# arnauqb/GradABM-JUNE

Hardware: AMD Instinct MI355X
Metric: simulation steps/sec (higher is better)
Workload: dtype f32

## Files before the change

### gradabm-june_amd/csrc/gj_tiled.h

```cpp
#pragma once
#include <hip/hip_runtime.h>
#include <stdint.h>

#include <type_traits>

#include "../../include/gradjune_hip.h"
#include "gj_device.h"

namespace gj {

constexpr int kTileThreads = 1024;
constexpr int kTileWaves = kTileThreads / kWave;
constexpr int kMaxSliceAgents = 19840;
constexpr int kUnroll = 8;
#ifndef GJ_UNROLL_NARROW
#define GJ_UNROLL_NARROW 16
#endif
constexpr int kUnrollNarrow = GJ_UNROLL_NARROW;
#ifndef GJ_VENUE_UNROLL
#define GJ_VENUE_UNROLL 2
#endif
constexpr int kVenueUnroll = GJ_VENUE_UNROLL;
#ifndef GJ_VENUE_UNROLL_C
#define GJ_VENUE_UNROLL_C GJ_VENUE_UNROLL
// ... 389 lines not shown
  for (int pass = 0; pass < 2; ++pass) {
    if (pass == 1 && !two_sources) break;
    bool any = false;
    for (int t = 0; t < A.n_sets; ++t)
      if (A.sets[t].active && !A.sets[t].presum && (!two_sources || A.sets[t].raw == pass)) any = true;
    if (!any) continue;
    if (pass == 1) __syncthreads();
    load_slice(lds_x, pass == 0 ? A.qtrans : A.trans, base, n_local, tid);
    __syncthreads();
    for (int t = 0; t < A.n_sets; ++t) {
      const TSetA& T = A.sets[t];
      if (!T.active || T.presum || (two_sources && T.raw != pass)) continue;
      if (T.wide == 2) {
        scatter_explicit<kUnroll>(T, lds_x, s, wave, lane);
      } else if (T.wide) {
        scatter_set<true>(T, lds_x, s, wave, lane);
      } else {
        scatter_set<false>(T, lds_x, s, wave, lane);
      }
    }
  }
}

struct TSetB {
  const int32_t* blk_v0;
  const int32_t* blk_e0;
  const uint16_t* e_lv;
  const uint8_t* e_cls;
  float* val;
  const float* v_pc;
  float* cum;
  int32_t stride;
  int32_t nk;
  float beta[GJ_MAX_NETS_PER_SET];
  int32_t table[GJ_MAX_NETS_PER_SET];
  int32_t age75[GJ_MAX_NETS_PER_SET];
  int32_t leisure;
  int32_t direct;
  uint32_t term_limit;
  int32_t _pad_b;
  const uint16_t* pv_blk;
  const int32_t* blk_r0;
  const float* x;
  int64_t n_x;
};

struct TileBArgs {
  TSetB sets[GJ_MAX_SETS];
  const int32_t* work;
  const float* tables;
  int32_t day_type;
  int32_t mode;
  int32_t transpose;
  int32_t _pad;
};

struct ClassWeights {
  float l, lw;
};
__device__ __forceinline__ ClassWeights class_weights(const float* tables, int table, int age75, int day_type, int c) {
  const float l = tables[(int64_t)table * GJ_TABLE_SIZE + day_type * 200 + c];
  return {l, age75 ? l * (((c % 100) > 75) ? 1.0f : 0.0f) : l};
}
template <bool TRANSMITTING, bool RECEIVING, typename TSet>
__device__ __forceinline__ void fill_class_weights(float* transmitting, float* receiving, const TSet& T, const float* tables,
                                                   int day_type, int transpose, int tid) {
  for (int i = tid; i < T.nk * 200; i += kTileThreads) {
    const int k = i / 200, c = i % 200;
    const ClassWeights w = class_weights(tables, T.table[k], T.age75[k], day_type, c);
    if (TRANSMITTING) transmitting[i] = transpose ? w.lw : w.l;
    if (RECEIVING) receiving[i] = transpose ? w.l : w.lw;
  }
}

__device__ __noinline__ void venue_group_slow(fx_t* sums, uint32_t* vflags, int words, uint32_t limit, int base_k, int l0,
                                              int l1, int l2, int l3, int l4, int l5, int l6, int l7, float x0, float x1,
                                              float x2, float x3, float x4, float x5, float x6, float x7) {
  const int lv[8] = {l0, l1, l2, l3, l4, l5, l6, l7};
  const float x[8] = {x0, x1, x2, x3, x4, x5, x6, x7};
#pragma unroll
  for (int q = 0; q < 8; ++q) {
    if (lv[q] == 0xFFFF) continue;
    if (abs_bits(x[q]) <= limit) {
      atomicAdd(&sums[base_k + lv[q]], to_fx<kFxVenue>(x[q]));
    } else {
      fx_flag(vflags, words, base_k + lv[q], x[q]);
    }
  }
}

__device__ __forceinline__ int class_byte(uint32_t four, int j) { return (four >> (8 * j)) & 0xFF; }

struct Group8 {
  uint32_t w[4], c[2];
  float v[8];
  __device__ __forceinline__ Group8(uint4 raw, uint2 craw, float4 xa = make_float4(0.0f, 0.0f, 0.0f, 0.0f),
                                    float4 xb = make_float4(0.0f, 0.0f, 0.0f, 0.0f))
      : w{raw.x, raw.y, raw.z, raw.w}, c{craw.x, craw.y}, v{xa.x, xa.y, xa.z, xa.w, xb.x, xb.y, xb.z, xb.w} {}
  __device__ __forceinline__ int lv(int q) const { return (w[q >> 1] >> ((q & 1) * 16)) & 0xFFFF; }
  __device__ __forceinline__ float x(int q) const { return v[q]; }
  __device__ __forceinline__ int cls(int q) const { return class_byte(c[q >> 2], q & 3); }
  __device__ __forceinline__ void drop(int q) { w[q >> 1] |= 0xFFFFu << ((q & 1) * 16); }
  __device__ __forceinline__ bool one_venue() const {
    return (w[0] == w[1]) && (w[1] == w[2]) && (w[2] == w[3]) && ((w[0] >> 16) == (w[0] & 0xFFFFu)) && (lv(0) != 0xFFFF);
  }
  __device__ __forceinline__ Group8 weighted(const float* tk) const {
    Group8 g = *this;
#pragma unroll
    for (int q = 0; q < 8; ++q) g.v[q] = tk[cls(q)] * v[q];
    return g;
  }
};

#ifdef GJ_DIAG_STAMPS
constexpr int kDiagVenueSlots = 8192;
__device__ unsigned long long gj_diag_venue[3 * kDiagVenueSlots];
struct VenueStamp {
  unsigned long long t0;
  __device__ VenueStamp() : t0(__builtin_amdgcn_s_memrealtime()) {}
  __device__ ~VenueStamp() {
    if (threadIdx.x == 0 && blockIdx.x < kDiagVenueSlots) {
      gj_diag_venue[3 * blockIdx.x] = t0;
      gj_diag_venue[3 * blockIdx.x + 1] = __builtin_amdgcn_s_memrealtime();
      gj_diag_venue[3 * blockIdx.x + 2] = __builtin_amdgcn_s_getreg((31 << 11) | 20) & 0xF;
    }
  }
};
#else
struct VenueStamp {};
#endif

struct VenueItem {
  const TSetB& T;
  int tid, nk;
  int v0, nv;
  int g0, g1;
  fx_t* sums;
  float* cumf;
  float* tabs;
  uint32_t* vflags;
  int vwords;
  int dummy;
  __device__ __forceinline__ VenueItem(const TSetB& T_, int j, float* lds, int tid_)
      : T(T_), tid(tid_), nk(T_.nk), v0(T_.blk_v0[j]), nv(T_.blk_v0[j + 1] - v0), g0(T_.blk_e0[j] >> 3),
        g1(T_.blk_e0[j + 1] >> 3), sums(reinterpret_cast<fx_t*>(lds)), cumf(lds), tabs(lds + 2 * ((size_t)nk * nv + 64)),
        vflags(reinterpret_cast<uint32_t*>(tabs + (T_.leisure ? 2 * nk * 200 : 0))), vwords((nk * nv + 64 + 31) / 32),
        dummy(nk * nv + (tid_ & 63)) {}
  __device__ __forceinline__ const uint4* lv8() const { return reinterpret_cast<const uint4*>(T.e_lv); }
  __device__ __forceinline__ const uint2* cls8() const { return reinterpret_cast<const uint2*>(T.e_cls); }
  __device__ __forceinline__ float4* val4() const { return reinterpret_cast<float4*>(T.val); }
};

__device__ __forceinline__ void run_sums(const VenueItem& W, const Group8& G, int base_k, fx_t* sums, uint32_t* vflags) {
  const uint32_t kLimit = W.T.term_limit;
  static_assert(kFxVenue == 36, "term_limit is derived from 2^(50 - kFxVenue) (fill_set_b)");
  if (__builtin_expect(max_abs_bits(G.v) > kLimit, 0)) {
    venue_group_slow(sums, vflags, W.vwords, kLimit, base_k, G.lv(0), G.lv(1), G.lv(2), G.lv(3), G.lv(4), G.lv(5),
                     G.lv(6), G.lv(7), G.x(0), G.x(1), G.x(2), G.x(3), G.x(4), G.x(5), G.x(6), G.x(7));
    return;
  }
  fx_t s8 = 0;
#pragma unroll
  for (int q = 0; q < 8; ++q) {
    const fx_t f = to_fx<kFxVenue>(G.x(q));
    const bool first = (q == 0) || (G.lv(q) != G.lv(q - (q > 0)));
    s8 = first ? f : s8 + f;
    const bool last = (q == 7) || (G.lv(q + (q < 7)) != G.lv(q));
    const bool take = last && G.lv(q) != 0xFFFF;
    atomicAdd(&sums[take ? base_k + G.lv(q) : W.dummy], s8);
  }
}
__device__ __forceinline__ bool one_venue_sum(const VenueItem& W, const Group8& G, int target, fx_t* sums) {
  if (__builtin_amdgcn_ballot_w64(max_abs_bits(G.v) > W.T.term_limit) != 0ull) return false;
  fx_t s = 0;
#pragma unroll
  for (int q = 0; q < 8; ++q) s += to_fx<kFxVenue>(G.x(q));
  s = wave_sum<fx_t>(s);
  if ((W.tid & (kWave - 1)) == 0) atomicAdd(&sums[target], s);
  return true;
}

__device__ __forceinline__ void venue_zero(const VenueItem& W, fx_t* sums, uint32_t* vflags) {
  for (int i = W.tid; i < W.nk * W.nv + 64; i += kTileThreads) sums[i] = 0;
  for (int i = W.tid; i < 2 * W.vwords; i += kTileThreads) vflags[i] = 0u;
}

__device__ __forceinline__ void venue_sums_tiled(const VenueItem& W, const float* weights, fx_t* sums, uint32_t* vflags) {
  const TSetB& T = W.T;
  auto add_group = [&](const Group8& G) {
    const bool mine = G.one_venue() && (G.lv(0) == __builtin_amdgcn_readfirstlane(G.lv(0)));
    const bool one_venue = __builtin_amdgcn_ballot_w64(mine) == ~0ull;
    if (!T.leisure) {
      if (!(one_venue && one_venue_sum(W, G, G.lv(0), sums))) run_sums(W, G, 0, sums, vflags);
    } else {
      for (int k = 0; k < W.nk; ++k) {
        const Group8 Gk = G.weighted(weights + k * 200);
        if (!(one_venue && one_venue_sum(W, Gk, k * W.nv + G.lv(0), sums))) run_sums(W, Gk, k * W.nv, sums, vflags);
      }
    }
  };
  for (int g = W.g0 + W.tid; g < W.g1; g += kVenueUnroll * kTileThreads) {
    uint4 raw[kVenueUnroll];
    float4 xa[kVenueUnroll], xb[kVenueUnroll];
    uint2 craw[kVenueUnroll];
#pragma unroll
    for (int u = 0; u < kVenueUnroll; ++u) {
      const int gu = min(g + u * kTileThreads, W.g1 - 1);
      raw[u] = W.lv8()[gu];
      xa[u] = load_nt(W.val4() + 2 * gu);
      xb[u] = load_nt(W.val4() + 2 * gu + 1);
      craw[u] = T.leisure ? W.cls8()[gu] : make_uint2(0u, 0u);
    }
#pragma unroll
    for (int u = 0; u < kVenueUnroll; ++u)
      if (g + u * kTileThreads < W.g1) add_group(Group8(raw[u], craw[u], xa[u], xb[u]));
  }
}

__device__ __forceinline__ void venue_sums_runs(const VenueItem& W, int j, fx_t* sums, uint32_t* vflags) {
  const TSetB& T = W.T;
  const int r0 = T.blk_r0[j], r1 = T.blk_r0[j + 1];
  const uint4* pv8 = reinterpret_cast<const uint4*>(T.pv_blk);
  const float4* x4 = reinterpret_cast<const float4*>(T.x);
  const int ga = r0 >> 3, gb = (r1 + 7) >> 3;
  const int g_in = (int)(T.n_x >> 3);
  for (int g = ga + W.tid; g < gb; g += kVenueUnroll * kTileThreads) {
    uint4 raw[kVenueUnroll];
    float4 xa[kVenueUnroll], xb[kVenueUnroll];
#pragma unroll
    for (int u = 0; u < kVenueUnroll; ++u) {
      const int gu = min(g + u * kTileThreads, gb - 1);
      raw[u] = pv8[gu];
      if (gu < g_in) {
        xa[u] = x4[2 * gu];
        xb[u] = x4[2 * gu + 1];
      } else {
        float t[8];
#pragma unroll
        for (int q = 0; q < 8; ++q) t[q] = ((int64_t)gu * 8 + q < T.n_x) ? T.x[(int64_t)gu * 8 + q] : 0.0f;
        xa[u] = make_float4(t[0], t[1], t[2], t[3]);
        xb[u] = make_float4(t[4], t[5], t[6], t[7]);
      }
    }
#pragma unroll
    for (int u = 0; u < kVenueUnroll; ++u) {
      const int gu = g + u * kTileThreads;
      if (gu >= gb) continue;
      Group8 G(raw[u], make_uint2(0u, 0u), xa[u], xb[u]);
#pragma unroll
      for (int q = 0; q < 8; ++q) {
        const int a = gu * 8 + q;
        if (!(a >= r0 && a < r1)) G.drop(q);
      }
      run_sums(W, G, 0, sums, vflags);
    }
  }
}

__device__ __forceinline__ void venue_cum_write(const VenueItem& W, const fx_t* sums, const uint32_t* vflags, float* cumf) {
  const TSetB& T = W.T;
  for (int l0 = W.tid; l0 < W.nv; l0 += kCumBatch * kTileThreads) {
    float pc[kCumBatch];
#pragma unroll
    for (int u = 0; u < kCumBatch; ++u) pc[u] = T.v_pc[W.v0 + min(l0 + u * kTileThreads, W.nv - 1)];
    for (int k = 0; k < W.nk; ++k) {
      const float beta = T.beta[k];
#pragma unroll
      for (int u = 0; u < kCumBatch; ++u) {
        const int lv = l0 + u * kTileThreads;
        if (lv < W.nv) {
          const float c = (beta * pc[u]) * fx_read<kFxVenue>(sums, vflags, W.vwords, k * W.nv + lv);
          T.cum[(int64_t)(W.v0 + lv) * T.stride + k] = c;
          cumf[2 * (k * W.nv + lv)] = c;
        }
      }
    }
  }
}
__device__ __forceinline__ void venue_cum_read(const VenueItem& W, float* cumf) {
  const TSetB& T = W.T;
  for (int k = 0; k < W.nk; ++k) {
    for (int l0 = W.tid; l0 < W.nv; l0 += kCumBatch * kTileThreads) {
      float c[kCumBatch];
#pragma unroll
      for (int u = 0; u < kCumBatch; ++u)
        c[u] = T.cum[(int64_t)(W.v0 + min(l0 + u * kTileThreads, W.nv - 1)) * T.stride + k];
#pragma unroll
      for (int u = 0; u < kCumBatch; ++u) {
        const int lv = l0 + u * kTileThreads;
        if (lv < W.nv) cumf[2 * (k * W.nv + lv)] = c[u];
      }
    }
  }
}

__device__ __forceinline__ void venue_gather(const VenueItem& W, const float* weights, const float* cumf) {
  const TSetB& T = W.T;
  const int nk = W.nk, nv = W.nv;
  for (int g = W.g0 + W.tid; g < W.g1; g += kVenueUnrollC * kTileThreads) {
    uint4 raw[kVenueUnrollC];
    uint2 craw[kVenueUnrollC];
#pragma unroll
    for (int u = 0; u < kVenueUnrollC; ++u) {
      const int gu = min(g + u * kTileThreads, W.g1 - 1);
      raw[u] = W.lv8()[gu];
      craw[u] = T.leisure ? W.cls8()[gu] : make_uint2(0u, 0u);
    }
#pragma unroll
    for (int u = 0; u < kVenueUnrollC; ++u) {
      const int gu = g + u * kTileThreads;
      if (gu >= W.g1) continue;
      const Group8 G(raw[u], craw[u]);
      float r[8];
      if (!T.leisure) {
#pragma unroll
        for (int q = 0; q < 8; ++q) {
          const int lv = G.lv(q);
          const float c = cumf[2 * (lv != 0xFFFF ? lv : 0)];
          r[q] = (lv != 0xFFFF) ? c : 0.0f;
        }
      } else {
#pragma unroll
        for (int q = 0; q < 8; ++q) {
          const int lv = G.lv(q);
          const int c = G.cls(q);
          const int li = lv != 0xFFFF ? lv : 0;
          float a = 0.0f;
          for (int k = 0; k < nk; ++k) a += weights[k * 200 + c] * cumf[2 * (k * nv + li)];
          r[q] = (lv != 0xFFFF) ? a : 0.0f;
        }
      }
      store_nt(W.val4() + 2 * gu, make_float4(r[0], r[1], r[2], r[3]));
      store_nt(W.val4() + 2 * gu + 1, make_float4(r[4], r[5], r[6], r[7]));
    }
  }
}

#ifndef GJ_VENUE_WAVES_PER_SIMD
#define GJ_VENUE_WAVES_PER_SIMD 4
#endif
__global__ __launch_bounds__(kTileThreads, GJ_VENUE_WAVES_PER_SIMD) void k_tile_venues(const TileBArgs B) {
  extern __shared__ __align__(16) float lds_s[];
  [[maybe_unused]] const VenueStamp gj_stamp;
  const int set = B.work[2 * blockIdx.x], j = B.work[2 * blockIdx.x + 1];
  const TSetB& T = B.sets[set];
  if (T.nk == 0) return;
  const VenueItem W(T, j, lds_s, threadIdx.x);
  if (T.leisure) fill_class_weights<true, true>(W.tabs, W.tabs + W.nk * 200, T, B.tables, B.day_type, B.transpose, W.tid);
  if (B.mode != 2) {
    venue_zero(W, W.sums, W.vflags);
    __syncthreads();
    venue_sums_tiled(W, W.tabs, W.sums, W.vflags);
    if (T.pv_blk) venue_sums_runs(W, j, W.sums, W.vflags);
    __syncthreads();
    venue_cum_write(W, W.sums, W.vflags, W.cumf);
    if (B.mode == 1 || T.direct) return;
  } else {
    if (T.direct) return;
    venue_cum_read(W, W.cumf);
  }
  __syncthreads();
  venue_gather(W, W.tabs + W.nk * 200, W.cumf);
}

constexpr int GJ_MAX_PRESUM = 6;
constexpr int64_t kPresumBad = (int64_t)0x8000000000000000ll;
struct TPSet {
  const uint16_t* ell;
  int64_t plane_stride;
  fx_t* partial;
  int32_t planes, V, stride, nk;
  int32_t group_venues;
  int32_t raw, leisure, _pad;
  int32_t table[GJ_MAX_NETS_PER_SET];
  int32_t age75[GJ_MAX_NETS_PER_SET];
};
struct TilePArgs {
  TPSet sets[GJ_MAX_PRESUM];
  int32_t n_sets;
  int32_t agents_per_wg;
  int64_t n_agents;
  const float* trans;
  const float* qtrans;
  const uint8_t* cls;
  const float* tables;
  int32_t day_type, transpose;
};

constexpr int kPresumQuads = 3;
__device__ __forceinline__ void fx_add_or_poison(fx_t* sums, uint32_t* flags, int i, float x) {
  const bool ok = fabsf(x) <= fx_max<kFxVenue>();
  atomicAdd(&sums[i], to_fx<kFxVenue>(ok ? x : 0.0f));
  if (__builtin_expect(!ok, 0)) atomicOr(&flags[i >> 5], 1u << (i & 31));
}

__global__ __launch_bounds__(kTileThreads) void k_tile_presum(const TilePArgs P) {
  extern __shared__ __align__(16) fx_t lds_p[];
  const int tid = threadIdx.x;
  const int64_t a_begin = (int64_t)blockIdx.x * P.agents_per_wg;
  const int64_t a_end = min(P.n_agents, a_begin + P.agents_per_wg);
  const int n_quads = (int)((max(a_end - a_begin, (int64_t)0) + 3) >> 2);
  for (int t = 0; t < P.n_sets; ++t) {
    const TPSet& T = P.sets[t];
    const int nk = T.nk;
    const float* x = T.raw ? P.trans : P.qtrans;
    for (int v0 = 0; v0 < T.V; v0 += T.group_venues) {
      const int nv = min(T.group_venues, T.V - v0);
      const int n_sums = nv * nk;
      const int dummy = n_sums + (tid & 63);
      float* wtab = reinterpret_cast<float*>(lds_p + n_sums + 64);
      uint32_t* flags = reinterpret_cast<uint32_t*>(wtab + (T.leisure ? nk * 200 : 0));
      __syncthreads();
      for (int i = tid; i < n_sums + 64; i += kTileThreads) lds_p[i] = 0;
      for (int i = tid; i < (n_sums + 64 + 31) / 32; i += kTileThreads) flags[i] = 0u;
      if (T.leisure) fill_class_weights<true, false>(wtab, nullptr, T, P.tables, P.day_type, P.transpose, tid);
// ... 663 lines not shown
```

### gradabm-june_amd/csrc/gradjune_hip.hip

```cpp
#include <hip/hip_runtime.h>
#include <math.h>
#include <stdint.h>
#include <string.h>

#include "../../include/gradjune_hip.h"
#include "gj_device.h"
#include "gj_tiled.h"
#include "gj_agent.h"

namespace gj {

struct SetP1 {
  const int32_t* v_rowptr;
  const int32_t* v_agent;
  const float* v_pc;
  float* cum;
  int32_t stride;
  int32_t nk;
  float beta[GJ_MAX_NETS_PER_SET];
  int32_t table[GJ_MAX_NETS_PER_SET];
  int32_t raw;
  int32_t leisure;
};

struct P1Args {
  SetP1 sets[GJ_MAX_SETS];
  const gj_block* blocks;
  const float* trans;
  const float* qtrans;
  const uint8_t* cls;
  const float* tables;
  float* partial;
  int32_t day_type;
};

struct SetP2 {
  const int32_t* a_rowptr;
  const int32_t* a_venue;
  const float* cum;
  int32_t stride;
  int32_t nk;
  int32_t mask[GJ_MAX_NETS_PER_SET];
  int32_t table[GJ_MAX_NETS_PER_SET];
};

struct P2Args {
  SetP2 groups[GJ_MAX_SETS];
  int32_t n_groups;
  int32_t any_leisure;
  int64_t n_agents;
  const uint8_t* cls;
  const float* tables;
  const float* stage;
  float* susceptibility;
  float* is_infected;
  float* infection_time;
// ... 773 lines not shown
  for (int g = 0; g < G.n; ++g) {
    const int s = G.set[g];
    if (!uses_presum(plan, s)) continue;
    if (R.n_sets == GJ_MAX_PRESUM) return GJ_E_PLAN;
    PReduceSet& X = R.sets[R.n_sets++];
    const gj_edge_set& E = plan->sets[s];
    X.partial = reinterpret_cast<const fx_t*>(T->sets[s].presum);
    X.v_pc = E.v_pcontact;
    X.cum = E.cum;
    X.V = (int32_t)E.n_venues;
    X.stride = E.cum_stride;
    X.nk = G.nk[g];
    X.first = (int32_t)total;
    const NetGroup C = classify_group(p, G, g);
    memcpy(X.beta, C.beta, sizeof(X.beta));
    total += (int64_t)X.V * X.nk;
  }
  if (R.n_sets == 0 || total == 0) return GJ_OK;
  if (total > INT32_MAX) return GJ_E_RANGE;
  R.total = (int32_t)total;
  return launch(k_presum_reduce, grid_for(total, 0, kWave), kThreads, 0, stream, R);
}

static int tiled_scatter(const gj_plan* plan, const gj_agent_state* st, const gj_step_params* p, const Groups& G,
                         hipStream_t stream) {
  const gj_tiled* T = plan->tiled;
  if (plan->n_ext_agents == 0 || G.n == 0) return GJ_OK;
  TileAArgs A;
  fill_set_a(plan, p, G, A.sets);
  A.n_sets = plan->n_sets;
  A.slice_agents = T->slice_agents;
  A.n_agents = plan->n_ext_agents;
  A.trans = st->transmission;
  A.qtrans = p->has_quarantine ? st->q_transmission : st->transmission;
  const size_t lds = slice_lds(T, sizeof(float));
  int rc = allow_lds(k_tile_scatter, lds);
  if (rc) return rc;
  rc = launch(k_tile_scatter, T->n_slices, kTileThreads, lds, stream, A);
  if (rc) return rc;
  return tiled_presum(plan, st, p, G, stream);
}

static uint32_t venue_term_limit(int32_t max_venue_edges) {
  int e = 14;
  int64_t p2 = 4096;
  while (p2 < (int64_t)max_venue_edges && e > -20) {
    p2 <<= 1;
    --e;
  }
  const float lim = ldexpf(1.0f, e);
  uint32_t bits;
  memcpy(&bits, &lim, sizeof(bits));
  return bits;
}

static int tiled_venues(const gj_plan* plan, const gj_agent_state* st, const gj_step_params* p, const Groups& G, int mode,
                        hipStream_t stream) {
  const gj_tiled* T = plan->tiled;
  if (G.n == 0) return GJ_OK;
  if (T->n_work == 0) return mode == 2 ? GJ_OK : tiled_presum_reduce(plan, p, G, stream);
  TileBArgs B;
  for (int s = 0; s < GJ_MAX_SETS; ++s) B.sets[s] = TSetB{};
  size_t lds = 16;
  for (int g = 0; g < G.n; ++g) {
    const int s = G.set[g];
    const gj_tiled_set& S = T->sets[s];
    const gj_edge_set& E = plan->sets[s];
    TSetB& X = B.sets[s];
    X.blk_v0 = S.blk_v0;
    X.blk_e0 = S.blk_e0;
    X.e_lv = S.e_lv;
    X.e_cls = S.e_cls;
    X.val = S.val;
    X.v_pc = E.v_pcontact;
    X.cum = E.cum;
    X.stride = E.cum_stride;
    X.nk = S.n_blocks > 0 ? G.nk[g] : 0;
    if (uses_presum(plan, s)) X.nk = 0;
    X.direct = S.ell_k != 0;
    const NetGroup C = classify_group(p, G, g);
    X.leisure = C.leisure;
    memcpy(X.beta, C.beta, sizeof(X.beta));
    memcpy(X.table, C.table, sizeof(X.table));
    memcpy(X.age75, C.age75, sizeof(X.age75));
    if (C.leisure && !S.e_cls && E.n_edges > 0) return GJ_E_PLAN;
    if (const int rc = check_group(C)) return rc;
    X.pv_blk = nullptr;
    X.blk_r0 = nullptr;
    X.x = nullptr;
    X.n_x = 0;
    if (S.run_pv_blk && mode != 2) {
      if (X.leisure) return GJ_E_PLAN;
      X.x = (p->has_quarantine && !C.raw) ? st->q_transmission : st->transmission;
      if (!X.x) return GJ_E_NULL;
      if (!aligned16(X.x, S.run_pv_blk)) return GJ_E_PLAN;
      X.pv_blk = S.run_pv_blk;
      X.blk_r0 = S.run_blk_r0;
      X.n_x = plan->n_ext_agents;
    }
    const size_t n_sums = (size_t)X.nk * S.max_block_venues + 64;
    const size_t need = n_sums * sizeof(fx_t) + (X.leisure ? 2 * 200 * (size_t)X.nk : 0) * sizeof(float) +
                        2 * ((n_sums + 31) / 32 * 4);
    X.term_limit = venue_term_limit(S.max_venue_edges);
    if (X.nk && need > lds) lds = need;
  }
  B.work = T->work;
  B.tables = plan->tables;
  B.day_type = p->day_type;
  B.mode = mode;
  B.transpose = p->transpose;
  int rc = allow_lds(k_tile_venues, lds);
  if (rc) return rc;
  rc = launch(k_tile_venues, T->n_work, kTileThreads, lds, stream, B);
  if (rc || mode == 2) return rc;
  return tiled_presum_reduce(plan, p, G, stream);
}

static int tiled_agents(const gj_plan* plan, const gj_agent_state* st, const gj_step_params* p, const Groups& G,
                        const gj_step_io* io, int sample, hipStream_t stream) {
  const gj_tiled* T = plan->tiled;
  if (plan->n_agents == 0) return GJ_OK;
  TileDArgs D;
  fill_set_a(plan, p, G, D.sets);
  D.n_sets = plan->n_sets;
  D.slice_agents = T->slice_agents;
  D.n_agents = plan->n_agents;
  D.stage = st->current_stage;
  D.susceptibility = st->susceptibility;
  D.is_infected = st->is_infected;
  D.infection_time = st->infection_time;
  D.not_infected_probs = io ? io->not_infected_probs : nullptr;
  D.new_infected = io ? io->new_infected : nullptr;
  D.trans_susc = io ? io->trans_susc : nullptr;
  D.agent_sums = io ? io->agent_sums : nullptr;
  D.exp_noise = io ? io->exp_noise : nullptr;
  D.now = p->now;
  D.dt = p->delta_time;
  D.q_thr = p->q_threshold;
  D.has_q = p->has_quarantine;
  D.sample = sample;
  D.seed = p->seed;
  D.step = p->step;
  D.agent_offset = p->agent_offset;
  D.clock = p->clock;
  D.acc_scratch = T->agent_scratch;
  size_t lds = agents_lds(T);
  D.n_direct = 0;
  D.day_type = p->day_type;
  D.transpose = p->transpose;
  D.cls = plan->agent_class;
  D.tables = plan->tables;
  const int64_t owned_slices = (plan->n_agents + T->slice_agents - 1) / T->slice_agents;
  for (int g = 0; g < G.n; ++g) {
    const int s = G.set[g];
    const gj_tiled_set& S = T->sets[s];
    const gj_edge_set& E = plan->sets[s];
    const bool run = S.run_pv_win != nullptr;
    if ((!S.ell_k && !run) || S.n_blocks == 0 || E.n_edges == 0) continue;
    if (D.n_direct == GJ_MAX_DIRECT) return GJ_E_PLAN;
    TDirect& X = D.direct[D.n_direct++];
    X.ell = run ? S.run_pv_win : S.ell;
    X.cum = E.cum;
    X.planes = run ? 1 : S.ell_k / 2;
    X.plane_stride = owned_slices * (int64_t)T->slice_agents * 2;
    X.V = run ? S.run_max_window : (int32_t)E.n_venues;
    X.win_lo = run ? S.run_win_lo : nullptr;
// ... 38 lines not shown
    const size_t direct_lds = 4 * ((size_t)2 * kClassWeightFloats + (size_t)cap0 + kWave + (size_t)cap1 + kWave);
    if (direct_lds > lds) lds = direct_lds;
  }
  D.io_vec4 = aligned16(D.susceptibility, D.not_infected_probs, D.new_infected, D.trans_susc, D.acc_scratch, D.agent_sums);
  int rc = allow_lds(k_tile_agents, lds);
  if (rc) return rc;
  rc = launch(k_tile_agents, owned_slices, kTileThreads, lds, stream, D);
  if (rc || !D.acc_scratch) return rc;
  return launch(k_tile_epilogue, grid_for(plan->n_agents), kThreads, 0, stream, D);
}

static int check_symptoms(const uint8_t* agent_class, const float* new_infected, const float* current_stage,
                          const float* next_stage, const float* time_to_next_stage, const gj_symptoms_params* params,
                          const float* progresses, const float* dwell) {
  if (!agent_class || !new_infected || !current_stage || !next_stage || !time_to_next_stage || !params)
    return GJ_E_NULL;
  if (params->n_stages < 3 || params->n_stages > GJ_MAX_STAGES) return GJ_E_RANGE;
  if ((progresses == nullptr) != (dwell == nullptr)) return GJ_E_NULL;
  if (!progresses && !params->progress) return GJ_E_NULL;
  return GJ_OK;
}

static StatsArgs stats_args(int64_t n, const uint8_t* agent_class, const float* is_infected, const float* current_stage,
                            int32_t n_bins, const int32_t* bin_edges, int32_t dead_stage, double* out, bool vec4) {
  StatsArgs S;
  S.n = n;
  S.cls = agent_class;
  S.inf = is_infected;
  S.stage = current_stage;
  S.n_bins = n_bins;
  for (int b = 0; b <= GJ_MAX_AGE_BINS; ++b) S.edges[b] = (b <= n_bins) ? bin_edges[b] : 0;
  S.dead = dead_stage;
  S.vec4 = (vec4 && (uintptr_t)agent_class % 4 == 0) ? 1 : 0;
  S.out = out;
  return S;
}
static inline int64_t vec4_lanes(int64_t n, int vec4) { return vec4 ? (n >> 2) + 3 : n; }

static int check_profile_adjoint(const gj_agent_state* st, const float* trans_bar, const float* grad_inf_out,
                                 const float* grad_time_inout) {
  if (!st || !trans_bar || !grad_inf_out || !grad_time_inout) return GJ_E_NULL;
  if (!st->max_infectiousness || !st->shape || !st->rate || !st->shift || !st->infection_time || !st->is_infected)
    return GJ_E_NULL;
  return GJ_OK;
}

}


extern "C" {

#ifdef GJ_DIAG_STAMPS
int gj_diag_venue_stamps(unsigned long long* host_out) {
  return (int)hipMemcpyFromSymbol(host_out, HIP_SYMBOL(gj::gj_diag_venue), sizeof(unsigned long long) * 3 * gj::kDiagVenueSlots);
}
#endif

int gj_version(void) { return GJ_ABI_VERSION; }

const char* gj_error_string(int code) {
  switch (code) {
    case GJ_OK: return "ok";
    case GJ_E_NULL: return "required pointer is NULL";
    case GJ_E_RANGE: return "count or index out of range";
    case GJ_E_PLAN: return "inconsistent plan or network list";
    case GJ_E_NODEVICE: return "no HIP device, or not a gfx950 (MI355X) device";
    default: break;
  }
  if (code > 0) return hipGetErrorString((hipError_t)code);
  return "unknown error";
}

int gj_check_device(void) {
  int dev = 0;
  if (hipGetDevice(&dev) != hipSuccess) return GJ_E_NODEVICE;
  hipDeviceProp_t prop;
  if (hipGetDeviceProperties(&prop, dev) != hipSuccess) return GJ_E_NODEVICE;
  const char* want = "gfx950";
  for (int i = 0; want[i]; ++i)
    if (prop.gcnArchName[i] != want[i]) return GJ_E_NODEVICE;
  return GJ_OK;
}

int gj_transmission_update(const gj_plan* plan, const gj_agent_state* state, const gj_step_params* params,
                           void* stream) {
  int rc = gj::check_plan(plan);
  if (rc) return rc;
  if (!params) return GJ_E_NULL;
  rc = gj::check_state(plan, state, params);
  if (rc) return rc;
  return gj::do_transmission(plan, state, params, (hipStream_t)stream);
}

int gj_quarantine_transmission(const gj_plan* plan, const gj_agent_state* state, const gj_step_params* params,
                               void* stream) {
  int rc = gj::check_plan(plan);
  if (rc) return rc;
  if (!params) return GJ_E_NULL;
  rc = gj::check_state(plan, state, params, false);
  if (rc) return rc;
  if (!params->has_quarantine || plan->n_agents == 0) return GJ_OK;
  const int64_t n = plan->n_agents;
  return gj::launch(gj::k_quarantine_transmission, gj::grid_for(n), gj::kThreads, 0, (hipStream_t)stream, n,
                    state->current_stage, state->transmission, state->q_transmission, params->q_threshold);
}

int gj_venue_reduce(const gj_plan* plan, const gj_agent_state* state, const gj_step_params* params, void* stream) {
  int rc = gj::check_plan(plan);
  if (rc) return rc;
// ... 478 lines not shown
```

### gradabm-june_amd/grad_june_amd/_native.py

```python
from __future__ import annotations

import ctypes as C
import os
from typing import Optional

GJ_ABI_VERSION = 7
GJ_MAX_SETS = 12
GJ_MAX_NETS = 16
GJ_MAX_NETS_PER_SET = 8
GJ_TABLE_SIZE = 400
GJ_ADJ_BETA_BLOCKS = 256
GJ_STREAM_EDGES = 2048
GJ_MAX_GROUPS = 1 << 28
GJ_GROUP_ERR_LABEL, GJ_GROUP_ERR_VALUE = 1, 2
GJ_SEED_CHUNK = 1024
GJ_STAGE_ERR_LABEL, GJ_STAGE_ERR_STAGE = 1, 2
GJ_STAGE_LDS_BINS, GJ_STAGE_ADJ_LDS_BINS = 8192, 2048
GJ_STAGE_LDS_THREADS, GJ_STAGE_LDS_BLOCKS = 1024, 512
GJ_STAGE_GLOBAL_THREADS, GJ_STAGE_GLOBAL_BLOCKS = 256, 2048
GJ_STAGE_LANE_LOADS = 63
GJ_STAGE_MAX_AGENTS = 1 << 40

MASK_RAW, MASK_Q, MASK_QL, MASK_QL_AGE75 = 0, 1, 2, 3

# ... 122 lines not shown
        ("transmission", _vp),
        ("q_transmission", _vp),
        ("current_stage", _vp),
    ]


class StepIO(C.Structure):
    _fields_ = [
        ("not_infected_probs", _vp),
        ("new_infected", _vp),
        ("exp_noise", _vp),
        ("trans_susc", _vp),
        ("agent_sums", _vp),
    ]


GJ_MAX_STAGES = 16


class SymptomsParams(C.Structure):
    _fields_ = [
        ("n_stages", C.c_int32),
        ("_pad", C.c_int32),
        ("progress", _vp),
        ("next_kind", C.c_int32 * GJ_MAX_STAGES),
        ("next_loc", C.c_float * GJ_MAX_STAGES),
        ("next_scale", C.c_float * GJ_MAX_STAGES),
        ("rec_kind", C.c_int32 * GJ_MAX_STAGES),
        ("rec_loc", C.c_float * GJ_MAX_STAGES),
        ("rec_scale", C.c_float * GJ_MAX_STAGES),
        ("time", C.c_float),
        ("_pad2", C.c_float),
        ("seed", C.c_uint64),
        ("step", C.c_uint64),
        ("agent_offset", C.c_int64),
    ]


class SeedPlan(C.Structure):
    _fields_ = [
        ("n_sorted", C.c_int64),
        ("n_chunks", C.c_int64),
        ("order", _vp),
        ("seg_offsets", _vp),
        ("chunk_first", _vp),
        ("chunk_group", _vp),
    ]


SYMBOLS = {
    "gj_version": (C.c_int, []),
    "gj_error_string": (C.c_char_p, [C.c_int]),
    "gj_check_device": (C.c_int, []),
    "gj_transmission_update": (C.c_int, [C.POINTER(Plan), C.POINTER(AgentState), C.POINTER(StepParams), _vp]),
    "gj_quarantine_transmission": (C.c_int, [C.POINTER(Plan), C.POINTER(AgentState), C.POINTER(StepParams), _vp]),
    "gj_venue_reduce": (C.c_int, [C.POINTER(Plan), C.POINTER(AgentState), C.POINTER(StepParams), _vp]),
    "gj_agent_gather": (
        C.c_int,
        [C.POINTER(Plan), C.POINTER(AgentState), C.POINTER(StepParams), C.POINTER(StepIO), C.c_int, _vp],
    ),
    "gj_sample_infect": (
        C.c_int,
        [C.c_int64, _vp, _vp, C.c_uint64, C.c_uint64, C.c_int64, C.c_float, _vp, _vp, _vp, _vp, _vp],
    ),
    "gj_adjoint_sample": (
        C.c_int,
        [C.c_int64, _vp, _vp, _vp, _vp, C.c_uint64, C.c_uint64, C.c_int64, C.c_float, C.c_float, _vp, _vp, _vp, _vp,
         _vp, _vp, _vp, _vp],
    ),
    "gj_adjoint_transmission": (C.c_int, [C.c_int64, C.POINTER(AgentState), C.c_float, _vp, _vp, _vp, _vp, _vp]),
    "gj_adjoint_transmission_params": (
        C.c_int, [C.c_int64, C.POINTER(AgentState), C.c_float, _vp, _vp, _vp, _vp, _vp, _vp, _vp, _vp, _vp]),
    "gj_adjoint_seed": (
        C.c_int,
        [C.c_int64, _vp, _vp, C.c_int32, C.POINTER(SeedPlan), _vp, _vp, _vp, C.c_uint64, C.c_uint64, C.c_int64,
         C.c_float, _vp, _vp, _vp, _vp, _vp, _vp, _vp, _vp, _vp, _vp],
    ),
    "gj_adjoint_beta_partial": (
        C.c_int,
        [C.c_int64, C.c_int32, C.c_int32, _vp, _vp, _vp, _vp, C.POINTER(C.c_float), C.POINTER(C.c_int32), _vp, _vp],
    ),
    "gj_adjoint_beta_finish": (C.c_int, [C.c_int32, _vp, _vp, _vp, _vp]),
    "gj_symptoms_update": (
        C.c_int,
        [C.c_int64, _vp, _vp, _vp, _vp, _vp, C.POINTER(SymptomsParams), _vp, _vp, _vp],
    ),
    "gj_adjoint_symptoms": (
        C.c_int,
        [C.c_int64, _vp, _vp, _vp, _vp, _vp, C.POINTER(SymptomsParams)] + [_vp] * 10,
    ),
    "gj_step_stats": (C.c_int, [C.c_int64, _vp, _vp, _vp, C.c_int32, C.POINTER(C.c_int32), C.c_int32, _vp, _vp]),
    "gj_group_stats": (C.c_int, [C.c_int64, _vp, C.c_int32, _vp, _vp, C.c_int32, _vp, _vp, _vp]),
    "gj_adjoint_group_stats": (C.c_int, [C.c_int64, _vp, C.c_int32, _vp, C.c_int32, _vp, _vp, _vp, _vp, _vp]),
    "gj_stage_stats": (C.c_int, [C.c_int64, _vp, C.c_int32, C.c_int32, _vp, _vp, _vp, _vp, _vp]),
    "gj_adjoint_stage_stats": (C.c_int, [C.c_int64, _vp, C.c_int32, C.c_int32, _vp, _vp, _vp, _vp, _vp, _vp]),
    "gj_step": (C.c_int, [C.POINTER(Plan), C.POINTER(AgentState), C.POINTER(StepParams), C.POINTER(StepIO), _vp]),
    "gj_step_phase": (
        C.c_int,
        [C.POINTER(Plan), C.POINTER(AgentState), C.POINTER(StepParams), C.POINTER(StepIO), C.c_int, _vp],
    ),
    "gj_clock_advance": (C.c_int, [_vp, C.c_double, _vp]),
    "gj_symptoms_step_stats": (
        C.c_int,
        [C.c_int64, _vp, _vp, _vp, _vp, _vp, C.POINTER(SymptomsParams), _vp, _vp, _vp, C.c_int32, C.POINTER(C.c_int32),
         C.c_int32, _vp, _vp],
    ),
# ... 93 lines not shown
```

### include/gradjune_hip.h

```cpp
#ifndef GRADJUNE_HIP_H
#define GRADJUNE_HIP_H

#include <stdint.h>

#ifdef __cplusplus
extern "C" {
#endif

#define GJ_ABI_VERSION 7

#define GJ_MAX_SETS 12
#define GJ_MAX_NETS 16
#define GJ_MAX_NETS_PER_SET 8
#define GJ_TABLE_SIZE 400

#define GJ_OK 0
#define GJ_E_NULL (-1)
#define GJ_E_RANGE (-2)
#define GJ_E_PLAN (-3)
#define GJ_E_NODEVICE (-4)

typedef enum gj_mask_kind {
  GJ_MASK_RAW = 0,
  GJ_MASK_Q = 1,
// ... 89 lines not shown
  int32_t _pad;
  const gj_tiled* tiled;
} gj_plan;

typedef struct gj_network {
  float beta;
  int32_t set;
  int32_t mask_kind;
  int32_t table;
} gj_network;

typedef struct gj_clock {
  float now;
  float _pad;
  uint64_t step;
  double now0;
  uint64_t step0;
} gj_clock;

typedef struct gj_step_params {
  float now;
  float delta_time;
  int32_t day_type;
  int32_t has_quarantine;
  float q_threshold;
  int32_t n_nets;
  uint64_t seed;
  uint64_t step;
  int64_t agent_offset;
  int32_t transpose;
  int32_t _pad;
  gj_network nets[GJ_MAX_NETS];
  const gj_clock* clock;
} gj_step_params;

typedef struct gj_agent_state {
  const float* max_infectiousness;
  const float* shape;
  const float* rate;
  const float* shift;
  float* infection_time;
  float* is_infected;
  float* susceptibility;
  float* transmission;
  float* q_transmission;
  const float* current_stage;
} gj_agent_state;

int gj_version(void);
const char* gj_error_string(int code);

int gj_check_device(void);

typedef struct gj_step_io {
  float* not_infected_probs;
  float* new_infected;
  const float* exp_noise;
  float* trans_susc;
  float* agent_sums;
} gj_step_io;

int gj_transmission_update(const gj_plan* plan, const gj_agent_state* state,
                           const gj_step_params* params, void* stream);

int gj_quarantine_transmission(const gj_plan* plan, const gj_agent_state* state,
                               const gj_step_params* params, void* stream);

int gj_venue_reduce(const gj_plan* plan, const gj_agent_state* state,
                    const gj_step_params* params, void* stream);

int gj_agent_gather(const gj_plan* plan, const gj_agent_state* state,
                    const gj_step_params* params, const gj_step_io* io, int sample,
                    void* stream);

int gj_sample_infect(int64_t n_agents, const float* not_infected_probs, const float* exp_noise,
                     uint64_t seed, uint64_t step, int64_t agent_offset, float now,
                     float* new_infected, float* susceptibility, float* is_infected,
                     float* infection_time, void* stream);

#define GJ_MAX_STAGES 16
typedef struct gj_symptoms_params {
  int32_t n_stages;
  int32_t _pad;
  const float* progress;
  int32_t next_kind[GJ_MAX_STAGES];
  float next_loc[GJ_MAX_STAGES];
  float next_scale[GJ_MAX_STAGES];
  int32_t rec_kind[GJ_MAX_STAGES];
  float rec_loc[GJ_MAX_STAGES];
  float rec_scale[GJ_MAX_STAGES];
  float time;
  float _pad2;
  uint64_t seed, step;
  int64_t agent_offset;
} gj_symptoms_params;

int gj_symptoms_update(int64_t n, const uint8_t* agent_class, const float* new_infected,
                       float* current_stage, float* next_stage, float* time_to_next_stage,
                       const gj_symptoms_params* params, const float* progresses, const float* dwell,
                       void* stream);

#define GJ_MAX_AGE_BINS 8
int gj_step_stats(int64_t n, const uint8_t* agent_class, const float* is_infected,
                  const float* current_stage, int32_t n_bins, const int32_t* bin_edges ,
                  int32_t dead_stage, double* out, void* stream);

// ... 158 lines not shown
```

Before: 1968.

## Make venue tile kernel persistent with atomic ticket work-stealing and prefetch

Converts the one-block-per-work-item venue kernel into a persistent kernel capped at the CU count. Blocks pull further items through a per-stream global atomic ticket counter, and the next item's header is prefetched in stages overlapped with the current item's gather. It also reuses the leisure class-weight tables across consecutive items from the same set and preloads the first cumulative and gather batches before barriers. This trades launch and tail overhead for extra atomics, additional LDS head slots and serialized work within each block. Persistence is skipped during graph capture.

Result: no change. 1978 (median of 2 runs) (+0.5%).

```diff
diff --git a/gradabm-june_amd/csrc/gj_tiled.h b/gradabm-june_amd/csrc/gj_tiled.h
--- a/gradabm-june_amd/csrc/gj_tiled.h
+++ b/gradabm-june_amd/csrc/gj_tiled.h
@@ -465,8 +465,13 @@
   int32_t day_type;
   int32_t mode;
   int32_t transpose;
+  int32_t pair;
+  int32_t n_work;
   int32_t _pad;
 };
+
+constexpr int kVenueTicketPairs = 64;
+__device__ unsigned int gj_venue_tickets[2 * kVenueTicketPairs];
 
 struct ClassWeights {
   float l, lw;
@@ -527,37 +532,66 @@
 
 #ifdef GJ_DIAG_STAMPS
 constexpr int kDiagVenueSlots = 8192;
-__device__ unsigned long long gj_diag_venue[3 * kDiagVenueSlots];
+constexpr int kDiagVenueWords = 8;
+__device__ unsigned long long gj_diag_venue[kDiagVenueWords * kDiagVenueSlots];
 struct VenueStamp {
-  unsigned long long t0;
-  __device__ VenueStamp() : t0(__builtin_amdgcn_s_memrealtime()) {}
-  __device__ ~VenueStamp() {
-    if (threadIdx.x == 0 && blockIdx.x < kDiagVenueSlots) {
-      gj_diag_venue[3 * blockIdx.x] = t0;
-      gj_diag_venue[3 * blockIdx.x + 1] = __builtin_amdgcn_s_memrealtime();
-      gj_diag_venue[3 * blockIdx.x + 2] = __builtin_amdgcn_s_getreg((31 << 11) | 20) & 0xF;
+  unsigned long long t[6];
+  __device__ __forceinline__ void start() {
+    t[0] = __builtin_amdgcn_s_memrealtime();
+#pragma unroll
+    for (int k = 1; k < 6; ++k) t[k] = 0;
+  }
+  __device__ __forceinline__ void mark(int k) { t[k] = __builtin_amdgcn_s_memrealtime(); }
+  __device__ __forceinline__ void mark_after(int k, uint32_t loaded) {
+    asm volatile("s_nop 0" ::"v"(loaded));
+    if (t[k] == 0) mark(k);
+  }
+  __device__ __forceinline__ void write(int item) {
+    if (threadIdx.x == 0 && item < kDiagVenueSlots) {
+      unsigned long long last = t[0];
+#pragma unroll
+      for (int k = 0; k < 6; ++k) {
+        last = t[k] ? t[k] : last;
+        gj_diag_venue[kDiagVenueWords * item + k] = last;
+      }
+      gj_diag_venue[kDiagVenueWords * item + 6] = __builtin_amdgcn_s_getreg((31 << 11) | 20) & 0xF;
+      gj_diag_venue[kDiagVenueWords * item + 7] = blockIdx.x;
     }
   }
 };
 #else
-struct VenueStamp {};
+struct VenueStamp {
+  __device__ __forceinline__ void start() {}
+  __device__ __forceinline__ void mark(int) {}
+  __device__ __forceinline__ void mark_after(int, uint32_t) {}
+  __device__ __forceinline__ void write(int) {}
+};
 #endif
+
+struct VenueHead {
+  int item, set, j;
+  int v0, nv;
+  int g0, g1;
+  int r0, r1;
+};
+constexpr int kVenueHeadInts = 16;
 
 struct VenueItem {
   const TSetB& T;
   int tid, nk;
   int v0, nv;
   int g0, g1;
+  int r0, r1;
+  float* tabs;
   fx_t* sums;
   float* cumf;
-  float* tabs;
   uint32_t* vflags;
   int vwords;
   int dummy;
-  __device__ __forceinline__ VenueItem(const TSetB& T_, int j, float* lds, int tid_)
-      : T(T_), tid(tid_), nk(T_.nk), v0(T_.blk_v0[j]), nv(T_.blk_v0[j + 1] - v0), g0(T_.blk_e0[j] >> 3),
-        g1(T_.blk_e0[j + 1] >> 3), sums(reinterpret_cast<fx_t*>(lds)), cumf(lds), tabs(lds + 2 * ((size_t)nk * nv + 64)),
-        vflags(reinterpret_cast<uint32_t*>(tabs + (T_.leisure ? 2 * nk * 200 : 0))), vwords((nk * nv + 64 + 31) / 32),
+  __device__ __forceinline__ VenueItem(const TSetB& T_, const VenueHead& H, float* lds, int tid_)
+      : T(T_), tid(tid_), nk(T_.nk), v0(H.v0), nv(H.nv), g0(H.g0), g1(H.g1), r0(H.r0), r1(H.r1), tabs(lds),
+        sums(reinterpret_cast<fx_t*>(lds + (T_.leisure ? 2 * nk * 200 : 0))), cumf(reinterpret_cast<float*>(sums)),
+        vflags(reinterpret_cast<uint32_t*>(sums + ((size_t)nk * nv + 64))), vwords((nk * nv + 64 + 31) / 32),
         dummy(nk * nv + (tid_ & 63)) {}
   __device__ __forceinline__ const uint4* lv8() const { return reinterpret_cast<const uint4*>(T.e_lv); }
   __device__ __forceinline__ const uint2* cls8() const { return reinterpret_cast<const uint2*>(T.e_cls); }
@@ -598,7 +632,8 @@
   for (int i = W.tid; i < 2 * W.vwords; i += kTileThreads) vflags[i] = 0u;
 }
 
-__device__ __forceinline__ void venue_sums_tiled(const VenueItem& W, const float* weights, fx_t* sums, uint32_t* vflags) {
+__device__ __forceinline__ void venue_sums_tiled(const VenueItem& W, const float* weights, fx_t* sums, uint32_t* vflags,
+                                                 VenueStamp& stamp) {
   const TSetB& T = W.T;
   auto add_group = [&](const Group8& G) {
     const bool mine = G.one_venue() && (G.lv(0) == __builtin_amdgcn_readfirstlane(G.lv(0)));
@@ -624,15 +659,16 @@
       xb[u] = load_nt(W.val4() + 2 * gu + 1);
       craw[u] = T.leisure ? W.cls8()[gu] : make_uint2(0u, 0u);
     }
+    stamp.mark_after(1, raw[0].x);
 #pragma unroll
     for (int u = 0; u < kVenueUnroll; ++u)
       if (g + u * kTileThreads < W.g1) add_group(Group8(raw[u], craw[u], xa[u], xb[u]));
   }
 }
 
-__device__ __forceinline__ void venue_sums_runs(const VenueItem& W, int j, fx_t* sums, uint32_t* vflags) {
+__device__ __forceinline__ void venue_sums_runs(const VenueItem& W, fx_t* sums, uint32_t* vflags) {
   const TSetB& T = W.T;
-  const int r0 = T.blk_r0[j], r1 = T.blk_r0[j + 1];
+  const int r0 = W.r0, r1 = W.r1;
   const uint4* pv8 = reinterpret_cast<const uint4*>(T.pv_blk);
   const float4* x4 = reinterpret_cast<const float4*>(T.x);
   const int ga = r0 >> 3, gb = (r1 + 7) >> 3;
@@ -670,12 +706,27 @@
   }
 }
 
-__device__ __forceinline__ void venue_cum_write(const VenueItem& W, const fx_t* sums, const uint32_t* vflags, float* cumf) {
+struct CumBatch {
+  float pc[kCumBatch];
+};
+__device__ __forceinline__ void venue_cum_load(const VenueItem& W, int l0, CumBatch& P) {
+#pragma unroll
+  for (int u = 0; u < kCumBatch; ++u) P.pc[u] = W.T.v_pc[W.v0 + max(min(l0 + u * kTileThreads, W.nv - 1), 0)];
+}
+__device__ __forceinline__ void venue_cum_write(const VenueItem& W, const fx_t* sums, const uint32_t* vflags, float* cumf,
+                                                const CumBatch& first) {
   const TSetB& T = W.T;
   for (int l0 = W.tid; l0 < W.nv; l0 += kCumBatch * kTileThreads) {
     float pc[kCumBatch];
-#pragma unroll
-    for (int u = 0; u < kCumBatch; ++u) pc[u] = T.v_pc[W.v0 + min(l0 + u * kTileThreads, W.nv - 1)];
+    if (l0 == W.tid) {
+#pragma unroll
+      for (int u = 0; u < kCumBatch; ++u) pc[u] = first.pc[u];
+    } else {
+      CumBatch P;
+      venue_cum_load(W, l0, P);
+#pragma unroll
+      for (int u = 0; u < kCumBatch; ++u) pc[u] = P.pc[u];
+    }
     for (int k = 0; k < W.nk; ++k) {
       const float beta = T.beta[k];
 #pragma unroll
@@ -707,18 +758,103 @@
   }
 }
 
-__device__ __forceinline__ void venue_gather(const VenueItem& W, const float* weights, const float* cumf) {
+__device__ __forceinline__ VenueHead venue_head(const TileBArgs& B, int item) {
+  VenueHead H;
+  H.item = item;
+  H.set = B.work[2 * item];
+  H.j = B.work[2 * item + 1];
+  const TSetB& T = B.sets[H.set];
+  H.v0 = H.nv = H.g0 = H.g1 = H.r0 = H.r1 = 0;
+  if (T.nk == 0) return H;
+  H.v0 = T.blk_v0[H.j];
+  H.nv = T.blk_v0[H.j + 1] - H.v0;
+  H.g0 = T.blk_e0[H.j] >> 3;
+  H.g1 = T.blk_e0[H.j + 1] >> 3;
+  if (T.pv_blk) {
+    H.r0 = T.blk_r0[H.j];
+    H.r1 = T.blk_r0[H.j + 1];
+  }
+  return H;
+}
+
+struct NextItem {
+  const TileBArgs& B;
+  int* slot;
+  int stage;
+  unsigned int tk;
+  int item, s, j, v0, v1, e0, e1, r0, r1;
+  __device__ __forceinline__ NextItem(const TileBArgs& B_, int* slot_, bool on) : B(B_), slot(slot_), stage(on ? 0 : 4), tk(0u) {}
+  __device__ __forceinline__ void ticket() {
+    if (stage != 0) return;
+    if (threadIdx.x == 0) tk = atomicAdd(&gj_venue_tickets[2 * B.pair], 1u);
+    stage = 1;
+  }
+  __device__ __forceinline__ void work() {
+    if (stage != 1) return;
+    const unsigned int t = (unsigned int)__builtin_amdgcn_readfirstlane((int)tk);
+    item = (t < (unsigned int)B.n_work - gridDim.x) ? (int)(gridDim.x + t) : -1;
+    const int ic = max(item, 0);
+    s = B.work[2 * ic];
+    j = B.work[2 * ic + 1];
+    stage = 2;
+  }
+  __device__ __forceinline__ void blocks() {
+    if (stage != 2) return;
+    s = __builtin_amdgcn_readfirstlane(s);
+    j = __builtin_amdgcn_readfirstlane(j);
+    const TSetB& T = B.sets[s];
+    const int32_t* pv = T.nk ? T.blk_v0 + j : B.work;
+    const int32_t* pe = T.nk ? T.blk_e0 + j : B.work;
+    const int32_t* pr = (T.nk && T.pv_blk) ? T.blk_r0 + j : B.work;
+    v0 = pv[0], v1 = pv[1], e0 = pe[0], e1 = pe[1], r0 = pr[0], r1 = pr[1];
+    stage = 3;
+  }
+  __device__ __forceinline__ void publish() {
+    if (stage != 3) return;
+    if (threadIdx.x == 0) {
+      const TSetB& T = B.sets[s];
+      const bool live = T.nk != 0, runs = live && T.pv_blk;
+      slot[0] = item, slot[1] = s, slot[2] = j;
+      slot[3] = live ? v0 : 0, slot[4] = live ? v1 - v0 : 0;
+      slot[5] = live ? e0 >> 3 : 0, slot[6] = live ? e1 >> 3 : 0;
+      slot[7] = runs ? r0 : 0, slot[8] = runs ? r1 : 0;
+    }
+    stage = 4;
+  }
+  __device__ __forceinline__ void finish() {
+    ticket();
+    work();
+    blocks();
+    publish();
+  }
+  static __device__ __forceinline__ VenueHead read(const int* slot) {
+    VenueHead H;
+    H.item = slot[0], H.set = slot[1], H.j = slot[2], H.v0 = slot[3], H.nv = slot[4];
+    H.g0 = slot[5], H.g1 = slot[6], H.r0 = slot[7], H.r1 = slot[8];
+    return H;
+  }
+};
+
+struct GatherBatch {
+  uint4 raw[kVenueUnrollC];
+  uint2 craw[kVenueUnrollC];
+};
+__device__ __forceinline__ void venue_gather_load(const VenueItem& W, int g, GatherBatch& L) {
+#pragma unroll
+  for (int u = 0; u < kVenueUnrollC; ++u) {
+    const int gu = min(g + u * kTileThreads, W.g1 - 1);
+    L.raw[u] = W.lv8()[gu];
+    L.craw[u] = W.T.leisure ? W.cls8()[gu] : make_uint2(0u, 0u);
+  }
+}
+__device__ __forceinline__ void venue_gather(const VenueItem& W, const float* weights, const float* cumf, const GatherBatch& first,
+                                             NextItem& next, VenueStamp& stamp) {
   const TSetB& T = W.T;
   const int nk = W.nk, nv = W.nv;
-  for (int g = W.g0 + W.tid; g < W.g1; g += kVenueUnrollC * kTileThreads) {
-    uint4 raw[kVenueUnrollC];
-    uint2 craw[kVenueUnrollC];
-#pragma unroll
-    for (int u = 0; u < kVenueUnrollC; ++u) {
-      const int gu = min(g + u * kTileThreads, W.g1 - 1);
-      raw[u] = W.lv8()[gu];
-      craw[u] = T.leisure ? W.cls8()[gu] : make_uint2(0u, 0u);
-    }
+  auto batch = [&](int g, const GatherBatch& L) {
+    const uint4 (&raw)[kVenueUnrollC] = L.raw;
+    const uint2 (&craw)[kVenueUnrollC] = L.craw;
+    stamp.mark_after(4, raw[0].x);
 #pragma unroll
     for (int u = 0; u < kVenueUnrollC; ++u) {
       const int gu = g + u * kTileThreads;
@@ -746,7 +882,17 @@
       store_nt(W.val4() + 2 * gu, make_float4(r[0], r[1], r[2], r[3]));
       store_nt(W.val4() + 2 * gu + 1, make_float4(r[4], r[5], r[6], r[7]));
     }
-  }
+  };
+  constexpr int kStride = kVenueUnrollC * kTileThreads;
+  int g = W.g0 + W.tid;
+  if (g < W.g1) batch(g, first);
+  next.blocks();
+  for (g += kStride; g < W.g1; g += kStride) {
+    GatherBatch L;
+    venue_gather_load(W, g, L);
+    batch(g, L);
+  }
+  next.publish();
 }
 
 #ifndef GJ_VENUE_WAVES_PER_SIMD
@@ -754,26 +900,64 @@
 #endif
 __global__ __launch_bounds__(kTileThreads, GJ_VENUE_WAVES_PER_SIMD) void k_tile_venues(const TileBArgs B) {
   extern __shared__ __align__(16) float lds_s[];
-  [[maybe_unused]] const VenueStamp gj_stamp;
-  const int set = B.work[2 * blockIdx.x], j = B.work[2 * blockIdx.x + 1];
-  const TSetB& T = B.sets[set];
-  if (T.nk == 0) return;
-  const VenueItem W(T, j, lds_s, threadIdx.x);
-  if (T.leisure) fill_class_weights<true, true>(W.tabs, W.tabs + W.nk * 200, T, B.tables, B.day_type, B.transpose, W.tid);
-  if (B.mode != 2) {
-    venue_zero(W, W.sums, W.vflags);
+  const bool pulls = B.pair >= 0;
+  int* slot = reinterpret_cast<int*>(lds_s);
+  float* lds = lds_s + (pulls ? kVenueHeadInts : 0);
+  const bool wave0 = __builtin_amdgcn_readfirstlane((int)threadIdx.x / kWave) == 0;
+  VenueHead H = venue_head(B, blockIdx.x);
+  int tabs_set = -1;
+  while (true) {
+    VenueStamp stamp;
+    stamp.start();
+    const TSetB& T = B.sets[H.set];
+    NextItem next(B, slot, pulls && wave0);
+    if (T.nk != 0 && !(B.mode == 2 && T.direct)) {
+      const VenueItem W(T, H, lds, threadIdx.x);
+      if (T.leisure && tabs_set != H.set)
+        fill_class_weights<true, true>(W.tabs, W.tabs + W.nk * 200, T, B.tables, B.day_type, B.transpose, W.tid);
+      tabs_set = T.leisure ? H.set : -1;
+      const bool gathers = !(B.mode == 1 || T.direct) && W.g1 > W.g0;
+      GatherBatch first;
+      if (B.mode != 2) {
+        venue_zero(W, W.sums, W.vflags);
+        __syncthreads();
+        venue_sums_tiled(W, W.tabs, W.sums, W.vflags, stamp);
+        if (T.pv_blk) venue_sums_runs(W, W.sums, W.vflags);
+        stamp.mark(2);
+        CumBatch pc;
+        venue_cum_load(W, W.tid, pc);
+        __syncthreads();
+        next.ticket();
+        venue_cum_write(W, W.sums, W.vflags, W.cumf, pc);
+      } else {
+        next.ticket();
+        venue_cum_read(W, W.cumf);
+      }
+      next.work();
+      stamp.mark(3);
+      if (gathers) {
+        venue_gather_load(W, W.g0 + W.tid, first);
+        __syncthreads();
+        venue_gather(W, W.tabs + W.nk * 200, W.cumf, first, next, stamp);
+      }
+    } else if (pulls) {
+      __syncthreads();
+    }
+    next.finish();
+    stamp.mark(5);
+    stamp.write(H.item);
+    if (!pulls) return;
     __syncthreads();
-    venue_sums_tiled(W, W.tabs, W.sums, W.vflags);
-    if (T.pv_blk) venue_sums_runs(W, j, W.sums, W.vflags);
-    __syncthreads();
-    venue_cum_write(W, W.sums, W.vflags, W.cumf);
-    if (B.mode == 1 || T.direct) return;
-  } else {
-    if (T.direct) return;
-    venue_cum_read(W, W.cumf);
-  }
-  __syncthreads();
-  venue_gather(W, W.tabs + W.nk * 200, W.cumf);
+    H = NextItem::read(slot);
+    if (H.item < 0) break;
+  }
+  if (threadIdx.x == 0) {
+    unsigned int* pair = &gj_venue_tickets[2 * B.pair];
+    if (atomicAdd(&pair[1], 1u) == gridDim.x - 1) {
+      atomicExch(&pair[0], 0u);
+      atomicExch(&pair[1], 0u);
+    }
+  }
 }
 
 constexpr int GJ_MAX_PRESUM = 6;
diff --git a/gradabm-june_amd/csrc/gradjune_hip.hip b/gradabm-june_amd/csrc/gradjune_hip.hip
--- a/gradabm-june_amd/csrc/gradjune_hip.hip
+++ b/gradabm-june_amd/csrc/gradjune_hip.hip
@@ -2,6 +2,8 @@
 #include <math.h>
 #include <stdint.h>
 #include <string.h>
+
+#include <mutex>
 
 #include "../../include/gradjune_hip.h"
 #include "gj_device.h"
@@ -881,6 +883,60 @@
   uint32_t bits;
   memcpy(&bits, &lim, sizeof(bits));
   return bits;
+}
+
+#ifndef GJ_VENUE_PERSISTENT
+#define GJ_VENUE_PERSISTENT 1
+#endif
+static std::mutex g_venue_mutex;
+static int g_venue_workgroups = 0;
+static hipStream_t g_venue_streams[kVenueTicketPairs];
+static int g_venue_n_streams = 0;
+constexpr int kMaxDevices = 64;
+static int g_device_cus[kMaxDevices];
+
+static int venue_ticket_pair(hipStream_t stream) {
+  std::lock_guard<std::mutex> lock(g_venue_mutex);
+  for (int i = 0; i < g_venue_n_streams; ++i)
+    if (g_venue_streams[i] == stream) return i;
+  if (g_venue_n_streams == kVenueTicketPairs) return -1;
+  g_venue_streams[g_venue_n_streams] = stream;
+  return g_venue_n_streams++;
+}
+static int device_cus() {
+  int dev = 0;
+  if (hipGetDevice(&dev) != hipSuccess || dev < 0 || dev >= kMaxDevices) return 0;
+  std::lock_guard<std::mutex> lock(g_venue_mutex);
+  if (g_device_cus[dev] == 0) {
+    hipDeviceProp_t prop;
+    if (hipGetDeviceProperties(&prop, dev) != hipSuccess) return 0;
+    g_device_cus[dev] = prop.multiProcessorCount;
+  }
+  return g_device_cus[dev];
+}
+static void venue_grid(int n_work, hipStream_t stream, size_t& lds, int64_t& grid, int& pair) {
+  grid = n_work;
+  pair = -1;
+  int knob;
+  {
+    std::lock_guard<std::mutex> lock(g_venue_mutex);
+    knob = g_venue_workgroups;
+  }
+  if (knob == 0 && !GJ_VENUE_PERSISTENT) knob = -1;
+  const size_t head = kVenueHeadInts * sizeof(int);
+  if (knob < 0 || lds + head > 160 * 1024) return;
+  hipStreamCaptureStatus capturing = hipStreamCaptureStatusNone;
+  if (hipStreamIsCapturing(stream, &capturing) != hipSuccess) {
+    (void)hipGetLastError();
+    return;
+  }
+  if (capturing != hipStreamCaptureStatusNone) return;
+  const int cap = knob > 0 ? knob : device_cus();
+  if (cap < 1) return;
+  pair = venue_ticket_pair(stream);
+  if (pair < 0) return;
+  grid = n_work < cap ? n_work : cap;
+  lds += head;
 }
 
 static int tiled_venues(const gj_plan* plan, const gj_agent_state* st, const gj_step_params* p, const Groups& G, int mode,
@@ -938,9 +994,13 @@
   B.day_type = p->day_type;
   B.mode = mode;
   B.transpose = p->transpose;
+  B.n_work = T->n_work;
+  B._pad = 0;
+  int64_t grid;
+  venue_grid(T->n_work, stream, lds, grid, B.pair);
   int rc = allow_lds(k_tile_venues, lds);
   if (rc) return rc;
-  rc = launch(k_tile_venues, T->n_work, kTileThreads, lds, stream, B);
+  rc = launch(k_tile_venues, grid, kTileThreads, lds, stream, B);
   if (rc || mode == 2) return rc;
   return tiled_presum_reduce(plan, p, G, stream);
 }
@@ -1085,9 +1145,17 @@
 
 #ifdef GJ_DIAG_STAMPS
 int gj_diag_venue_stamps(unsigned long long* host_out) {
-  return (int)hipMemcpyFromSymbol(host_out, HIP_SYMBOL(gj::gj_diag_venue), sizeof(unsigned long long) * 3 * gj::kDiagVenueSlots);
+  return (int)hipMemcpyFromSymbol(host_out, HIP_SYMBOL(gj::gj_diag_venue),
+                                  sizeof(unsigned long long) * gj::kDiagVenueWords * gj::kDiagVenueSlots);
 }
 #endif
+
+int gj_venue_workgroups(int n) {
+  if (n < -1) return GJ_E_RANGE;
+  std::lock_guard<std::mutex> lock(gj::g_venue_mutex);
+  gj::g_venue_workgroups = n;
+  return GJ_OK;
+}
 
 int gj_version(void) { return GJ_ABI_VERSION; }
 
diff --git a/gradabm-june_amd/grad_june_amd/_native.py b/gradabm-june_amd/grad_june_amd/_native.py
--- a/gradabm-june_amd/grad_june_amd/_native.py
+++ b/gradabm-june_amd/grad_june_amd/_native.py
@@ -198,6 +198,7 @@
     "gj_version": (C.c_int, []),
     "gj_error_string": (C.c_char_p, [C.c_int]),
     "gj_check_device": (C.c_int, []),
+    "gj_venue_workgroups": (C.c_int, [C.c_int]),
     "gj_transmission_update": (C.c_int, [C.POINTER(Plan), C.POINTER(AgentState), C.POINTER(StepParams), _vp]),
     "gj_quarantine_transmission": (C.c_int, [C.POINTER(Plan), C.POINTER(AgentState), C.POINTER(StepParams), _vp]),
     "gj_venue_reduce": (C.c_int, [C.POINTER(Plan), C.POINTER(AgentState), C.POINTER(StepParams), _vp]),
diff --git a/include/gradjune_hip.h b/include/gradjune_hip.h
--- a/include/gradjune_hip.h
+++ b/include/gradjune_hip.h
@@ -165,6 +165,8 @@
 
 int gj_check_device(void);
 
+int gj_venue_workgroups(int n);
+
 typedef struct gj_step_io {
   float* not_infected_probs;
   float* new_infected;
```
